# Chenxu1103/UNET-

Measured on AMD Instinct MI355X. Metric: frames/sec 512x512 3-class UNet++ inference; mask vs CPU reference, higher is better.
Workload: dtype f16 (MFMA operands split hi+lo, 3 MFMAs per product, f32 accumulate); 1 GPU; UNet++ 3-class 512x512 batch=16/GPU fp16-MFMA on 1 MI355X, synthetic frames, f32 NCHW in HBM -> uint8 mask in HBM; arch=nested, precision=exact, frames_per_gpu=16, global_batch=16, micro_batch=16, parallelism=frame-sharded x1, weights replicated (RCCL bcast)

## Files before the change

__graft_entry__.py:

```python
import os
import sys

ROOT = os.path.dirname(os.path.abspath(__file__))
if ROOT not in sys.path:
    sys.path.insert(0, ROOT)


def build() -> None:
    import unet_amd.nested_unet
    from unet_amd import _lib
    path = _lib.build(force=bool(os.environ.get("UNETPP_FORCE_BUILD")), verbose=True)
    import ctypes
    _lib.share_torch_hip_runtime()
    lib = ctypes.CDLL(path)
    for sym in _lib.ABI_SYMBOLS:
        getattr(lib, sym)
    print("built", path, "-", lib.unetpp_version.__name__, "ok")


def smoke() -> None:
    import numpy as np
    import torch
    from unet_amd import synthetic
    from unet_amd.nested_unet import NestedUNet
    sys.path.insert(0, os.path.join(ROOT, "oracle"))
    import unetpp_oracle as oracle

    assert torch.cuda.is_available(), "smoke() needs a HIP device"
    sd = synthetic.make_state_dict(3, 3, True, 2)
    frames = synthetic.make_frames_u8(2, 64, 96, "smooth", 7)
    x = synthetic.frames_to_chw_f32(frames)
    ref = oracle.torch_forward(sd, x)
    ref_mask, _, _ = oracle.masks_from_logits(ref)
    model = NestedUNet(3, deep_supervision=True, pretrained_encoder=False, max_batch=2, max_hw=(64, 96)).to("cuda:0")
    model.load_state_dict(sd, strict=True)
    model.eval()
    xt = torch.from_numpy(x).to("cuda:0")
    mask, logits = model.segment(xt, return_logits=True)
    torch.cuda.synchronize()
    err = float(np.abs(logits.cpu().numpy() - ref).max())
    margin = oracle.top2_margin(ref)
    bad = (mask.cpu().numpy() != ref_mask) & (margin > 1e-4)
    print(f"smoke: max|dlogit|={err:.3e} mask mismatches outside near-ties={int(bad.sum())}")
    assert err < 1e-3 and not bad.any()
    m8 = NestedUNet(3, deep_supervision=True, precision="exact8", max_batch=2, max_hw=(64, 96)).to("cuda:0")
    m8.load_state_dict(sd, strict=True)
    mask8, logits8 = m8.eval().segment(xt, return_logits=True)
    torch.cuda.synchronize()
    err8 = float(np.abs(logits8.cpu().numpy() - ref).max())
    bad8 = (mask8.cpu().numpy() != ref_mask) & (margin > 2 * err8 + 1e-7)
    print(f"smoke exact8: max|dlogit|={err8:.3e} mask mismatches outside near-ties={int(bad8.sum())}")
    assert err8 < 1e-3 and not bad8.any()


if __name__ == "__main__":
    build()
    if len(sys.argv) > 1 and sys.argv[1] == "smoke":
        smoke()
```

unet-_amd/_lib.py:

```python
from __future__ import annotations

import ctypes
import hashlib
import os
import shutil
import subprocess

_HERE = os.path.dirname(os.path.abspath(__file__))
LIB_PATH = os.path.join(_HERE, "libunetpp_hip.so")
CSRC = os.path.join(_HERE, "csrc")
SOURCES = ["unetpp_abi.hip"]
HEADERS = ["conv3x3_mfma.h", "conv3x3_ws.h", "tapmm_ws.h", "convt2x2_mfma.h", "aux_kernels.h", "components.h", "morphology.h", os.path.join("..", "..", "include", "unetpp.h")]

ABI_SYMBOLS = [
    "unetpp_create", "unetpp_destroy", "unetpp_last_error", "unetpp_version", "unetpp_weights_blob_bytes",
    "unetpp_weights_blob_bytes_arch",
    "unetpp_load_weights", "unetpp_load_weights_device", "unetpp_forward", "unetpp_forward_ex", "unetpp_mask_stats", "unetpp_workspace_bytes",
    "unetpp_resize_linear_u8", "unetpp_resize_nearest_roi_u8", "unetpp_status",
    "unetpp_profile_enable", "unetpp_profile_count", "unetpp_profile_read", "unetpp_profile_name",
    "unetpp_profile_work", "unetpp_debug_read", "unetpp_debug_keep_intermediates",
    "unetpp_ds_blob_bytes", "unetpp_load_ds_heads", "unetpp_forward_ds",
    "unetpp_components_workspace_bytes", "unetpp_components", "unetpp_components_filter",
    "unetpp_morphology", "unetpp_morphology_layout",
]

STATUS_OVERFLOW, STATUS_NAN = 1, 2
PREC_EXACT, PREC_FAST, PREC_EXACT8 = 0, 1, 2
PRECISIONS = {"exact": PREC_EXACT, "fast": PREC_FAST, "exact8": PREC_EXACT8}
ARCH_NESTED, ARCH_SIMPLE = 0, 1
IN_F32_NCHW, IN_U8_NHWC_BGR = 0, 1


class Config(ctypes.Structure):
    _fields_ = [("num_classes", ctypes.c_int), ("in_channels", ctypes.c_int), ("max_batch", ctypes.c_int),
                ("max_h", ctypes.c_int), ("max_w", ctypes.c_int), ("precision", ctypes.c_int),
                ("device", ctypes.c_int), ("micro_batch", ctypes.c_int), ("streams", ctypes.c_int), ("arch", ctypes.c_int)]


class CcRule(ctypes.Structure):
    _fields_ = [(n, ctypes.c_double) for n in ("min_area", "min_width", "max_width", "min_height_ratio", "min_aspect",
                                               "max_center_offset", "roi_width")]


CC_RULES = {"largest": 0, "spatial": 1, "cable_shape": 2}


class MorphElement(ctypes.Structure):
    _fields_ = [("kw", ctypes.c_int), ("kh", ctypes.c_int), ("ax", ctypes.c_int), ("ay", ctypes.c_int),
                ("host_data", ctypes.c_void_p)]


class MorphStep(ctypes.Structure):
    _fields_ = [(n, ctypes.c_int) for n in ("op", "dst", "a", "b", "element", "iterations")]


MORPH_OPS = {"dilate": 0, "erode": 1, "and": 2, "andnot": 3, "or": 4, "copy": 5}
RULES = {"argmax": 0, "thresholded_argmax": 1, "strict_bg_check": 2, "exclusive": 3}


class Outputs(ctypes.Structure):
    _fields_ = [("dev_logits", ctypes.c_void_p), ("dev_probs", ctypes.c_void_p), ("dev_mask", ctypes.c_void_p),
                ("dev_cable", ctypes.c_void_p), ("dev_tape", ctypes.c_void_p), ("rule", ctypes.c_int),
                ("t_cable", ctypes.c_float), ("t_tape", ctypes.c_float), ("bg_margin", ctypes.c_float),
                ("ct_margin", ctypes.c_float)]


CXXFLAGS = ["--offload-arch=gfx950", "-O3", "-std=c++17", "-fno-slp-vectorize"]


def source_hash() -> str:
    h = hashlib.sha256()
    h.update(" ".join(CXXFLAGS).encode() + b"\0")
    for rel in sorted(SOURCES + HEADERS):
        with open(os.path.join(CSRC, rel), "rb") as f:
            h.update(rel.encode() + b"\0" + f.read() + b"\0")
    return h.hexdigest()[:16]


def built_hash(path: str = LIB_PATH):
    try:
        with open(path, "rb") as f:
            blob = f.read()
    except OSError:
        return None
    i = blob.find(b"(gfx950) src:")
    if i < 0:
        return None
    tag = blob[i + 13:i + 13 + 16]
    if blob[i + 29:i + 36] == b" +wsdbg" and not os.environ.get("UNETPP_ALLOW_DBG_LIB"):
        return "wsdbg-build"
    return tag.decode("ascii", "replace")


def _stale() -> bool:
    return built_hash() != source_hash()


def _hipcc():
    cand = os.environ.get("HIPCC", "/opt/rocm/bin/hipcc")
    return cand if os.path.exists(cand) else shutil.which("hipcc")


def build(force: bool = False, verbose: bool = False) -> str:
    if not force and not _stale():
        return LIB_PATH
    hipcc = _hipcc()
    if not hipcc:
        raise RuntimeError("hipcc not found: cannot build libunetpp_hip.so")
    tmp = f"{LIB_PATH}.{os.getpid()}.tmp"
    cmd = [hipcc] + CXXFLAGS + ["-shared", "-fPIC", f'-DUNETPP_SRC_HASH="{source_hash()}"',
           "-o", tmp] + [os.path.join(CSRC, s) for s in SOURCES]
    if verbose:
        print(" ".join(cmd).replace(tmp, LIB_PATH), flush=True)
    try:
        subprocess.run(cmd, check=True, cwd=CSRC)
        os.replace(tmp, LIB_PATH)
    finally:
        if os.path.exists(tmp):
            os.remove(tmp)
    return LIB_PATH


_lib = None


def share_torch_hip_runtime() -> None:
    try:
        import torch
    except ImportError:
        pass


def load(build_if_missing: bool = True) -> ctypes.CDLL:
    global _lib
    if _lib is not None:
        return _lib
    share_torch_hip_runtime()
    if _stale():
        what = "is missing" if not os.path.exists(LIB_PATH) else f"was built from other sources (src:{built_hash()}, tree {source_hash()})"
        if not build_if_missing or not _hipcc():
            raise RuntimeError(f"{LIB_PATH} {what}: build it with __graft_entry__.build(); there is no CPU fallback")
        build()
    lib = ctypes.CDLL(LIB_PATH)
    vp, ci, cs = ctypes.c_void_p, ctypes.c_int, ctypes.c_size_t
    lib.unetpp_create.argtypes = [ctypes.POINTER(Config), ctypes.POINTER(vp)]; lib.unetpp_create.restype = ci
    lib.unetpp_destroy.argtypes = [vp]; lib.unetpp_destroy.restype = None
    lib.unetpp_last_error.argtypes = [vp]; lib.unetpp_last_error.restype = ctypes.c_char_p
    lib.unetpp_version.argtypes = []; lib.unetpp_version.restype = ctypes.c_char_p
    lib.unetpp_weights_blob_bytes.argtypes = [ci, ci]; lib.unetpp_weights_blob_bytes.restype = cs
    lib.unetpp_weights_blob_bytes_arch.argtypes = [ci, ci, ci]; lib.unetpp_weights_blob_bytes_arch.restype = cs
    lib.unetpp_load_weights.argtypes = [vp, vp, cs]; lib.unetpp_load_weights.restype = ci
    lib.unetpp_load_weights_device.argtypes = [vp, vp, cs, vp]; lib.unetpp_load_weights_device.restype = ci
    lib.unetpp_forward.argtypes = [vp, vp, ci, ci, ci, ci, vp, vp, vp, vp, vp]; lib.unetpp_forward.restype = ci
    lib.unetpp_forward_ex.argtypes = [vp, vp, ci, ci, ci, ci, ctypes.POINTER(Outputs), vp]; lib.unetpp_forward_ex.restype = ci
    lib.unetpp_mask_stats.argtypes = [vp, vp, ci, ci, ci, vp, vp, vp, vp]; lib.unetpp_mask_stats.restype = ci
    lib.unetpp_resize_linear_u8.argtypes = [vp, vp, ci, ci, ci, ci, vp, ci, ci, vp]; lib.unetpp_resize_linear_u8.restype = ci
    lib.unetpp_resize_nearest_roi_u8.argtypes = [vp, vp, ci, ci, ci, ci, vp, ci, ci, ci, ci, ci, ci, vp]
    lib.unetpp_resize_nearest_roi_u8.restype = ci
    lib.unetpp_workspace_bytes.argtypes = [vp]; lib.unetpp_workspace_bytes.restype = cs
    lib.unetpp_status.argtypes = [vp, ctypes.POINTER(ctypes.c_uint32), ci]; lib.unetpp_status.restype = ci
    lib.unetpp_profile_enable.argtypes = [vp, ci]; lib.unetpp_profile_enable.restype = ci
    lib.unetpp_profile_count.argtypes = [vp]; lib.unetpp_profile_count.restype = ci
    lib.unetpp_profile_read.argtypes = [vp, ctypes.POINTER(ctypes.c_float), ci]; lib.unetpp_profile_read.restype = ci
    lib.unetpp_profile_name.argtypes = [vp, ci]; lib.unetpp_profile_name.restype = ctypes.c_char_p
    lib.unetpp_profile_work.argtypes = [vp, ci, ctypes.POINTER(ctypes.c_double), ctypes.POINTER(ctypes.c_double)]
    lib.unetpp_profile_work.restype = ci
    lib.unetpp_debug_read.argtypes = [vp, ctypes.c_char_p, ctypes.POINTER(ctypes.c_float), cs]
    lib.unetpp_debug_read.restype = ctypes.c_longlong
    lib.unetpp_debug_keep_intermediates.argtypes = [vp, ci]; lib.unetpp_debug_keep_intermediates.restype = ci
    lib.unetpp_ds_blob_bytes.argtypes = [ci]; lib.unetpp_ds_blob_bytes.restype = cs
    lib.unetpp_load_ds_heads.argtypes = [vp, vp, cs]; lib.unetpp_load_ds_heads.restype = ci
    lib.unetpp_forward_ds.argtypes = [vp, vp, ci, ci, ci, ci, ctypes.POINTER(ctypes.POINTER(Outputs)), vp]
    lib.unetpp_forward_ds.restype = ci
# ... 18 lines not shown
```

unet-_amd/csrc/tapmm_ws.h:

```cpp
#pragma once
#include "conv3x3_ws.h"

namespace unetpp {

struct TapmmArgs {
  const half_t* low;
  const half_t* wpk;
  float* y;
  int N, hw, K, Nv;
#ifdef UNETPP_WS_DBG
  int dbg;
#endif
};

struct TapmmCfg {
  static constexpr int NT = 512, NCONS = 4, NPROD = 4;
  static constexpr int TM = 256, TN = 128, MT = 4, NTL = 2;
  static constexpr int A_BYTES = TM * 64, B_BYTES = TN * 64, STAGE_BYTES = A_BYTES + B_BYTES;
  static constexpr int SLOTS = 6, LDS_BYTES = SLOTS * STAGE_BYTES;
  static constexpr int A_PIECES = A_BYTES / 1024, B_PIECES = B_BYTES / 1024;
  static constexpr int A_IT = A_PIECES / NPROD, B_IT = B_PIECES / NPROD, DMA_PER_STAGE = A_IT + B_IT;
  static constexpr int AHEAD = 4;
  static_assert(LDS_BYTES <= 160 * 1024 && AHEAD + 2 <= SLOTS, "ring");
};

template <bool X8>
__global__ __launch_bounds__(512, 2) void tapmm_ws_kernel(TapmmArgs a) {
  using C = TapmmCfg;
  extern __shared__ __attribute__((aligned(16))) char smem[];
  touch_kernarg_lines<TapmmArgs>();
  const int tid = threadIdx.x, lane = tid & 63;
  const int wave = __builtin_amdgcn_readfirstlane(tid >> 6);
  const unsigned lds_base = (unsigned)(unsigned long)(lds_char_t*)smem;
  const int mtiles_img = (a.hw + C::TM - 1) / C::TM;
  const int ntiles = a.Nv / C::TN;
  const int total_tiles = a.N * mtiles_img * ntiles;
  const int nst = a.K / 16;
  const int G = (int)gridDim.x;
  const int slot = (G % 8 == 0) ? ((int)blockIdx.x % 8) * (G / 8) + (int)blockIdx.x / 8 : (int)blockIdx.x;
  auto decode = [&](int t, int& n, int& q0, int& vt) {
    vt = t % ntiles; t /= ntiles;
    const int mt = t % mtiles_img;
    n = t / mtiles_img;
    q0 = mt * C::TM;
  };
  if (slot >= total_tiles) return;
  if (wave >= C::NCONS) {
    const int pw = wave - C::NCONS;
    constexpr unsigned OOB = 0x80000000u;
    const unsigned blk_bytes = (unsigned)a.hw * 64u;
    int it_tile = slot, it_s = 0;
    int in_, iq0, ivt;
    decode(it_tile, in_, iq0, ivt);
    auto issue = [&](int ring) {
#ifdef UNETPP_WS_DBG
      if (a.dbg & 1) { if (++it_s == nst) { it_s = 0; it_tile += G; if (it_tile < total_tiles) decode(it_tile, in_, iq0, ivt); } return; }
#endif
      const __amdgpu_buffer_rsrc_t rs = __builtin_amdgcn_make_buffer_rsrc(
          (void*)(a.low + (size_t)in_ * (a.K / 16) * a.hw * 32), 0, (int)((a.K / 16) * blk_bytes), 0x00020000);
      const unsigned dstA = lds_base + ring * C::STAGE_BYTES;
#pragma unroll
      for (int it = 0; it < C::A_IT; ++it) {
        const int piece = pw + it * C::NPROD;
        const int q = iq0 + piece * 16 + (lane & 15);
        const unsigned voff = q < a.hw ? (unsigned)q * 64u + (unsigned)(lane >> 4) * 16u : OOB;
        blds16(rs, voff, it_s * (int)blk_bytes, dstA + piece * 1024);
      }
      const char* wsrc = (const char*)a.wpk + ((size_t)ivt * nst + it_s) * C::B_BYTES;
#pragma unroll
      for (int it = 0; it < C::B_IT; ++it) {
        const int piece = pw + it * C::NPROD;
        glds16(wsrc + piece * 1024, lane * 16, dstA + C::A_BYTES + piece * 1024);
      }
      if (++it_s == nst) {
        it_s = 0; it_tile += G;
        if (it_tile < total_tiles) decode(it_tile, in_, iq0, ivt);
      }
    };
    int issued = 0, g = 0;
    for (int k = 0; k <= C::AHEAD && it_tile < total_tiles; ++k, ++issued) issue(issued % C::SLOTS);
    for (int tile = slot; tile < total_tiles; tile += G)
      for (int s = 0; s < nst; ++s, ++g) {
        const int later = issued - (g + 2);
        if (later >= 3) asm volatile("s_waitcnt vmcnt(18)" ::: "memory");
        else if (later == 2) asm volatile("s_waitcnt vmcnt(12)" ::: "memory");
        else if (later == 1) asm volatile("s_waitcnt vmcnt(6)" ::: "memory");
        else asm volatile("s_waitcnt vmcnt(0)" ::: "memory");
        lds_barrier();
        if (it_tile < total_tiles) { issue(issued % C::SLOTS); ++issued; }
      }
    return;
  }

  const int cw = wave, pxh = cw & 1, vh = cw >> 1;
  static_assert(C::DMA_PER_STAGE == 6, "vmcnt ladder above");
  int a_off[C::MT];
#pragma unroll
  for (int mt = 0; mt < C::MT; ++mt) {
    const int px = pxh * 128 + mt * 32 + (lane & 31);
    a_off[mt] = (px >> 4) * 1024 + ((lane >> 5) * 16 + (px & 15)) * 16;
  }
  const int b_off = C::A_BYTES + (vh * 2) * 2048 + (lane >> 5) * 512 + (lane & 31) * 16;
  struct Frag { half8 ah[C::MT], al[C::MT], bh[C::NTL], bl[C::NTL]; };
  auto load_frags = [&](Frag& f, int ring) {
    const char* st = smem + ring * C::STAGE_BYTES;
#pragma unroll
    for (int mt = 0; mt < C::MT; ++mt) { f.ah[mt] = *(const half8*)(st + a_off[mt]); f.al[mt] = *(const half8*)(st + a_off[mt] + 512); }
#pragma unroll
    for (int nt = 0; nt < C::NTL; ++nt) { f.bh[nt] = *(const half8*)(st + b_off + nt * 2048); f.bl[nt] = *(const half8*)(st + b_off + nt * 2048 + 1024); }
  };
  float16v acc[C::MT][C::NTL];
  auto run_mfma = [&](const Frag& f) {
#ifdef UNETPP_WS_DBG
    if (a.dbg & 2) return;
#endif
#pragma unroll
    for (int mt = 0; mt < C::MT; ++mt)
#pragma unroll
      for (int nt = 0; nt < C::NTL; ++nt) {
        acc[mt][nt] = __builtin_amdgcn_mfma_f32_32x32x16_f16(f.bh[nt], f.al[mt], acc[mt][nt], 0, 0, 0);
        acc[mt][nt] = __builtin_amdgcn_mfma_f32_32x32x16_f16(f.bl[nt], f.ah[mt], acc[mt][nt], 0, 0, 0);
        acc[mt][nt] = __builtin_amdgcn_mfma_f32_32x32x16_f16(f.bh[nt], f.ah[mt], acc[mt][nt], 0, 0, 0);
      }
  };

  int g = 0;
  Frag f0, f1;
  bool have_f0 = false;
  struct HFrag { half8 a[C::MT], b[C::NTL]; };
  HFrag h0, h1;
  int8v xa[C::MT], xb[C::NTL];
  auto load_h = [&](HFrag& f, int ring) {
    const char* st = smem + ring * C::STAGE_BYTES;
#pragma unroll
    for (int mt = 0; mt < C::MT; ++mt) f.a[mt] = *(const half8*)(st + a_off[mt]);
#pragma unroll
    for (int nt = 0; nt < C::NTL; ++nt) f.b[nt] = *(const half8*)(st + b_off + nt * 2048);
  };
  auto load_x = [&](int ring0, int ring1) {
    const char* s0 = smem + ring0 * C::STAGE_BYTES;
    const char* s1 = smem + ring1 * C::STAGE_BYTES;
#pragma unroll
    for (int mt = 0; mt < C::MT; ++mt) {
      const int4v lo = *(const int4v*)(s0 + a_off[mt] + 512), hi = *(const int4v*)(s1 + a_off[mt] + 512);
      xa[mt] = __builtin_shufflevector(lo, hi, 0, 1, 2, 3, 4, 5, 6, 7);
    }
#pragma unroll
    for (int nt = 0; nt < C::NTL; ++nt) {
      const int4v lo = *(const int4v*)(s0 + b_off + nt * 2048 + 1024), hi = *(const int4v*)(s1 + b_off + nt * 2048 + 1024);
      xb[nt] = __builtin_shufflevector(lo, hi, 0, 1, 2, 3, 4, 5, 6, 7);
    }
  };
  auto main_mfma = [&](const HFrag& f) {
#pragma unroll
    for (int mt = 0; mt < C::MT; ++mt)
#pragma unroll
      for (int nt = 0; nt < C::NTL; ++nt) acc[mt][nt] = __builtin_amdgcn_mfma_f32_32x32x16_f16(f.b[nt], f.a[mt], acc[mt][nt], 0, 0, 0);
  };
  auto cross_mfma = [&]() {
#pragma unroll
    for (int mt = 0; mt < C::MT; ++mt)
#pragma unroll
      for (int nt = 0; nt < C::NTL; ++nt) {
        acc[mt][nt] = __builtin_amdgcn_mfma_scale_f32_32x32x64_f8f6f4(xb[nt], xa[mt], acc[mt][nt], 0 , 1 , 0, X8_SCALE_W, 0, X8_SCALE_A);
      }
  };
  for (int tile = slot; tile < total_tiles; tile += G) {
    int n, q0, vt;
    decode(tile, n, q0, vt);
#pragma unroll
    for (int mt = 0; mt < C::MT; ++mt)
#pragma unroll
      for (int nt = 0; nt < C::NTL; ++nt)
#pragma unroll
        for (int r = 0; r < 16; ++r) acc[mt][nt][r] = 0.f;
    const bool last_tile = tile + G >= total_tiles;
    if constexpr (X8) {
      for (int s = 0; s < nst; s += 2) {
        lds_barrier();
        if (!have_f0) { load_h(h0, g % C::SLOTS); have_f0 = true; }
        load_x(g % C::SLOTS, (g + 1) % C::SLOTS);
        load_h(h1, (g + 1) % C::SLOTS);
        __builtin_amdgcn_sched_barrier(0);
        main_mfma(h0);
        __builtin_amdgcn_sched_barrier(0);
        ++g;
        lds_barrier();
        const bool more = !(last_tile && s + 2 >= nst);
        if (more) load_h(h0, (g + 1) % C::SLOTS);
        have_f0 = more;
        __builtin_amdgcn_sched_barrier(0);
        cross_mfma();
        main_mfma(h1);
        __builtin_amdgcn_sched_barrier(0);
        ++g;
      }
    } else
    for (int s = 0; s < nst; s += 2) {
      lds_barrier();
      if (!have_f0) { load_frags(f0, g % C::SLOTS); have_f0 = true; }
      load_frags(f1, (g + 1) % C::SLOTS);
      __builtin_amdgcn_sched_barrier(0);
      run_mfma(f0);
      __builtin_amdgcn_sched_barrier(0);
      ++g;
      lds_barrier();
      const bool more = !(last_tile && s + 2 >= nst);
      if (more) load_frags(f0, (g + 1) % C::SLOTS);
      have_f0 = more;
      __builtin_amdgcn_sched_barrier(0);
      run_mfma(f1);
      __builtin_amdgcn_sched_barrier(0);
      ++g;
    }
#ifdef UNETPP_WS_DBG
    if (a.dbg & 4) { if (acc[0][0][0] == 12345.f) a.y[0] = 1.f; continue; }
#endif
    const int h = lane >> 5;
#pragma unroll
    for (int mt = 0; mt < C::MT; ++mt) {
      const int q = q0 + pxh * 128 + mt * 32 + (lane & 31);
#pragma unroll
      for (int nt = 0; nt < C::NTL; ++nt) {
        const int vb = vt * (C::TN / 32) + vh * 2 + nt;
        float* dst = a.y + (((size_t)n * (a.Nv / 32) + vb) * a.hw + q) * 32 + 4 * h;
        if (q < a.hw) {
#pragma unroll
          for (int qq = 0; qq < 4; ++qq) {
            typedef __attribute__((ext_vector_type(4))) float f32x4;
            *(f32x4*)(dst + 8 * qq) = (f32x4){acc[mt][nt][4 * qq], acc[mt][nt][4 * qq + 1], acc[mt][nt][4 * qq + 2], acc[mt][nt][4 * qq + 3]};
          }
        }
      }
    }
  }
}

__global__ void tapw_pack_kernel(const float* __restrict__ w, const float* __restrict__ mult, int Cout, int Cs, int Cup,
                                 half_t* __restrict__ out, long long units, int x8) {
  const long long u = (long long)blockIdx.x * blockDim.x + threadIdx.x;
  if (u >= units) return;
  long long t = u;
  const int vv = t % 32; t /= 32;
  const int kg = t % 2; t /= 2;
  const int pl = t % 2; t /= 2;
  const int vt = t % 4; t /= 4;
  const int nst = Cup / 16;
  const int ks = t % nst; t /= nst;
  const int v128 = (int)t;
  const int v = v128 * 128 + vt * 32 + vv;
  const int tap = v / Cout, co = v - tap * Cout;
  half8 r;
  float val[8];
#pragma unroll
  for (int e = 0; e < 8; ++e) {
    const int c = ks * 16 + kg * 8 + e;
    val[e] = w[((size_t)co * (Cs + Cup) + Cs + c) * 9 + tap] * mult[co];
    const half_t hi = (half_t)val[e];
    r[e] = pl == 0 ? hi : (half_t)(val[e] - (float)hi);
  }
  if (x8 && pl == 1) {
    unsigned wd[4];
#pragma unroll
    for (int q = 0; q < 2; ++q) {
      int a8 = 0, b8 = 0;
      float hi4[4], lo4[4];
#pragma unroll
      for (int i = 0; i < 4; ++i) { hi4[i] = val[4 * q + i] * 0.015625f; lo4[i] = (val[4 * q + i] - (float)(half_t)val[4 * q + i]) * 32.0f; }
      a8 = __builtin_amdgcn_cvt_pk_fp8_f32(hi4[0], hi4[1], a8, false); a8 = __builtin_amdgcn_cvt_pk_fp8_f32(hi4[2], hi4[3], a8, true);
      b8 = __builtin_amdgcn_cvt_pk_fp8_f32(lo4[0], lo4[1], b8, false); b8 = __builtin_amdgcn_cvt_pk_fp8_f32(lo4[2], lo4[3], b8, true);
      wd[2 * q] = (unsigned)a8; wd[2 * q + 1] = (unsigned)b8;
    }
    *(u32x4*)(out + u * 8) = (u32x4){wd[0], wd[1], wd[2], wd[3]};
    return;
  }
  *(half8*)(out + u * 8) = r;
}

struct UpsumArgs {
  const float* y;
  float* z;
  int N, H, W, Cout;
};

template <int TH_>
struct UpsumCfgT {
  static constexpr int TH = TH_, TW = 32, RH = TH / 2 + 3, RW = TW / 2 + 3, RECS = RH * RW;
  static constexpr int PIECES = (RECS * 128 + 1023) / 1024, BUF_BYTES = PIECES * 1024;
  static constexpr int YTAB_BYTES = (TH + 2) * 16, LDS_BYTES = BUF_BYTES + YTAB_BYTES;
  static constexpr int ITERS = (PIECES + 3) / 4;
};
typedef UpsumCfgT<16> UpsumCfg;

template <int TB, int TH_ = 16>
__global__ __launch_bounds__(256, TB == 1 ? 4 : 1) void upsum_kernel(UpsumArgs a) {
  using C = UpsumCfgT<TH_>;
  typedef __attribute__((ext_vector_type(4))) float f32x4;
  extern __shared__ __attribute__((aligned(16))) char smem[];
  const int H = a.H, W = a.W, h = H >> 1, w = W >> 1;
  const int tid = threadIdx.x, lane = tid & 63;
  const int wave = __builtin_amdgcn_readfirstlane(tid >> 6);
  const unsigned lds_base = (unsigned)(unsigned long)(lds_char_t*)smem;
  const int tiles_x = (W + C::TW - 1) / C::TW, tiles_y = (H + C::TH - 1) / C::TH;
  int t = blockIdx.x;
  const int tx = t % tiles_x; t /= tiles_x;
  const int ty = t % tiles_y; t /= tiles_y;
  const int cb = t % (a.Cout / 32);
  const int n = t / (a.Cout / 32);
  const int y0 = ty * C::TH, x0 = tx * C::TW;
  const float sh = h > 1 ? (float)(h - 1) / (float)(H - 1) : 0.f;
  const float sw = w > 1 ? (float)(w - 1) / (float)(W - 1) : 0.f;
  const int ybase = (int)(sh * (float)max(y0 - 1, 0)), xbase = (int)(sw * (float)max(x0 - 1, 0));
  const int vblocks = 9 * a.Cout / 32;
  const size_t plane = (size_t)h * w * 128;
  unsigned voff[C::ITERS];
#pragma unroll
  for (int it = 0; it < C::ITERS; ++it) {
    const int rec = (wave + it * 4) * 8 + (lane >> 3);
    const int ry = rec / C::RW, rx = rec - ry * C::RW;
    const int yy = min(ybase + ry, h - 1), xx = min(xbase + rx, w - 1);
    voff[it] = (wave + it * 4 < C::PIECES) ? (unsigned)((yy * w + xx) * 128 + (lane & 7) * 16) : 0x80000000u;
  }
  auto stage = [&](int tap, int buf) {
    const int vb = (tap * a.Cout) / 32 + cb;
    const __amdgpu_buffer_rsrc_t rs = __builtin_amdgcn_make_buffer_rsrc((void*)((const char*)a.y + ((size_t)n * vblocks + vb) * plane), 0,
                                                                       (int)plane, 0x00020000);
#pragma unroll
    for (int it = 0; it < C::ITERS; ++it) {
      const int piece = wave + it * 4;
      if (piece < C::PIECES) blds16(rs, voff[it], 0, lds_base + buf * C::BUF_BYTES + piece * 1024);
    }
  };
  const int cq = tid & 7, col = tid >> 3;
  int xo0[3], xo1[3]; float xl0[3], xl1[3];
#pragma unroll
  for (int dx = 0; dx < 3; ++dx) {
    const int xx = x0 + col + dx - 1;
    const bool in = xx >= 0 && xx < W && x0 + col < W;
    const float fx = sw * (float)max(xx, 0);
    const int c0 = min((int)fx, w - 1), c1 = c0 + (c0 < w - 1 ? 1 : 0);
    const float l1 = fminf(fmaxf(fx - (float)c0, 0.f), 1.f);
    xo0[dx] = min(max(c0 - xbase, 0), C::RW - 1) * 128 + cq * 16;
    xo1[dx] = min(max(c1 - xbase, 0), C::RW - 1) * 128 + cq * 16;
    xl0[dx] = in ? 1.f - l1 : 0.f; xl1[dx] = in ? l1 : 0.f;
  }
  struct YRow { int o0, o1; float l0, l1; };
  YRow* ytab = (YRow*)(smem + TB * C::BUF_BYTES);
  if (tid < C::TH + 2) {
    const int yy = y0 + tid - 1;
    const bool in = yy >= 0 && yy < H;
    const float fy = sh * (float)max(yy, 0);
    const int r0 = min((int)fy, h - 1), r1 = r0 + (r0 < h - 1 ? 1 : 0);
    const float l1 = fminf(fmaxf(fy - (float)r0, 0.f), 1.f);
    YRow e;
    e.o0 = min(max(r0 - ybase, 0), C::RH - 1) * (C::RW * 128);
    e.o1 = min(max(r1 - ybase, 0), C::RH - 1) * (C::RW * 128);
    e.l0 = in ? 1.f - l1 : 0.f; e.l1 = in ? l1 : 0.f;
// ... 41 lines not shown
```

unet-_amd/csrc/unetpp_abi.hip:

```cpp
#include <hip/hip_runtime.h>

#include <algorithm>
#include <cmath>
#include <cstdarg>
#include <cstdio>
#include <cstdlib>
#include <cstring>
#include <string>
#include <map>
#include <mutex>
#include <set>
#include <tuple>
#include <utility>
#include <vector>

#include "../../include/unetpp.h"
#include "aux_kernels.h"
#include "components.h"
#include "conv3x3_mfma.h"
#include "conv3x3_ws.h"
#include "convt2x2_mfma.h"
#include "morphology.h"
#include "tapmm_ws.h"

using namespace unetpp;

namespace {

thread_local std::string g_create_error;

constexpr uint32_t BLOB_MAGIC = 0x50504e55u;
constexpr uint32_t DS_BLOB_MAGIC = 0x53444e55u;
constexpr int BLOB_VERSION = 1;
const int NB[5] = {32, 64, 128, 256, 512};
const int SB[4] = {64, 128, 256, 512};

struct Tensor {
  std::string name;
  size_t off = 0;
  int C = 0;
  int lvl = 0;
  bool virt = false;
};

struct ConvLayer {
  std::string name;
  int cin_real = 0;
  int cout = 0;
  int lvl = 0;
  int in = -1, in2 = -1, out = -1, pool = -1;
  bool do_pool = false;
  int zt = -1;
  int y_t = -1, low_t = -1;
  half_t* tapw = nullptr;
  bool c0f = false;
  bool upf = false;
  bool ws = false;
  size_t w_off = 0, b_off = 0;
  int KC = 16, NW = 1, MW = 2, WAVES = 8;
  int nchunks = 1;
  half_t* wpk = nullptr;
  float* scale = nullptr;
  float* mult = nullptr;
};

struct ConvTLayer {
  std::string name;
  int cin = 0, cout = 0, lvl = 0;
  int in = -1, out = -1;
  size_t w_off = 0, b_off = 0;
  half_t* wpk = nullptr;
  float* scale = nullptr;
  float* mult = nullptr;
};

enum OpKind { OP_CONVERT, OP_CONV, OP_UP, OP_CONVT, OP_HEAD, OP_TAPMM, OP_UPSUM, OP_DS };
struct Op {
  OpKind kind;
  int idx = -1;
  int out = -1;
  bool fuse_head = false;
};

struct ProfRec {
  std::string name;
  double flops = 0, bytes = 0;
  int ev0 = -1, ev1 = -1;
};

}

struct unetpp_engine {
  unetpp_config cfg{};
  int P = 2;
  bool x8 = false;
  int mb = 1;
  int num_cus = 256;
  std::string err;
  char* arena = nullptr;
  size_t arena_bytes = 0;
  float* blob = nullptr;
  size_t blob_floats = 0;
  bool weights_loaded = false;
  std::vector<Tensor> tensors;
  std::vector<ConvLayer> convs;
  std::vector<ConvTLayer> convts;
  std::vector<Op> ops;
// ... 844 lines not shown
          return L.ws ? launch_ws(LaunchCtx{e->cfg.device, e->num_cus, e->ksplit_max, e->ksplit_min_chunks, e->ksplit_gate}, P, e->x8, a, L.do_pool, head, L.upf, L.c0f, s)
                    : launch_conv(LaunchCtx{e->cfg.device, e->num_cus}, P, L, mw, a, head, s);
        });
#ifdef UNETPP_WS_DBG
        if (stamp_this && L.ws) {
          static int printed = 0;
          std::vector<unsigned long long> hs(1024 * 32 * 5);
          (void)hipStreamSynchronize(s);
          (void)hipMemcpy(hs.data(), stamp_buf, hs.size() * 8, hipMemcpyDeviceToHost);
          if (printed++ == 3) {
            double sum[32] = {0};
            int nwg = 0;
            for (int b = 0; b < 1024; ++b) { if (!hs[b * 32 + 1] && !hs[b * 32 + 16]) continue; ++nwg; for (int i = 0; i < 32; ++i) sum[i] += (double)hs[b * 32 + i]; }
            fprintf(stderr, "[stamps %s] %d workgroups, mean cycles per workgroup:\n  consumer: barrier %.0f  chunks %.0f  epilogue %.0f  init %.0f\n"
                            "  producer: skip issue %.0f wait %.0f barrier %.0f | up issue %.0f interp %.0f (reads %.0f arithmetic %.0f split+stores %.0f) wait %.0f barrier %.0f | setup %.0f\n", L.name.c_str(), nwg,
                    sum[0] / nwg, sum[1] / nwg, sum[2] / nwg, sum[3] / nwg, sum[16] / nwg, sum[17] / nwg, sum[18] / nwg, sum[19] / nwg, sum[20] / nwg, sum[24] / nwg, sum[25] / nwg, sum[26] / nwg, sum[21] / nwg, sum[22] / nwg, sum[23] / nwg);
            std::vector<double> bg, en;
            unsigned long long t0 = ~0ull;
            std::vector<double> cb, pe;
            for (int b = 0; b < 1024; ++b) if (hs[b * 32 + 6]) t0 = std::min(t0, hs[b * 32 + 6]);
            for (int b = 0; b < 1024; ++b) if (hs[b * 32 + 6]) {
              bg.push_back((hs[b * 32 + 6] - t0) * 0.01); en.push_back((hs[b * 32 + 5] - t0) * 0.01);
              cb.push_back((hs[b * 32 + 4] - t0) * 0.01); pe.push_back((hs[b * 32 + 16 + 12] - t0) * 0.01);
            }
            std::sort(bg.begin(), bg.end()); std::sort(en.begin(), en.end()); std::sort(cb.begin(), cb.end()); std::sort(pe.begin(), pe.end());
            if (!bg.empty()) fprintf(stderr, "  consumer loop begins p50 %.2f max %.2f | producer wave 0 ends p50 %.2f max %.2f\n", cb[cb.size() / 2], cb.back(), pe[pe.size() / 2], pe.back());
            if (a.dbg & 131072)
              for (int b : {0, 1, 100, 200}) {
                for (int role = 0; role < 2; ++role) {
                  fprintf(stderr, "  wg %3d %s:", b, role ? "producer" : "consumer");
                  const unsigned long long* ev = hs.data() + 1024 * 32 + ((size_t)b * 2 + role) * 64;
                  for (int i = 0; i < 60 && ev[i]; ++i) fprintf(stderr, " %d:%.2f", (int)(ev[i] >> 56), (double)((ev[i] & 0xffffffffffffffull) - t0) * 0.01);
                  fprintf(stderr, "\n");
                }
              }
            if (!bg.empty())
              fprintf(stderr, "  wall clock (us after the first workgroup's kernel entry): entry p50 %.2f p90 %.2f max %.2f | end min %.2f p50 %.2f p90 %.2f max %.2f\n",
                      bg[bg.size() / 2], bg[bg.size() * 9 / 10], bg.back(), en.front(), en[en.size() / 2], en[en.size() * 9 / 10], en.back());
          }
        }
#endif
      } else if (op.kind == OP_TAPMM || op.kind == OP_UPSUM) {
        const ConvLayer& L = e->convs[op.idx];
        const int H = h >> L.lvl, W = w >> L.lvl;
        const int cs = e->tensors[L.in].C, cup = L.cin_real - cs;
        if (op.kind == OP_TAPMM) {
          TapmmArgs t{};
          t.low = tp(L.low_t); t.wpk = L.tapw; t.y = (float*)tp(L.y_t);
          t.N = nb; t.hw = (H >> 1) * (W >> 1); t.K = cup; t.Nv = 9 * L.cout;
#ifdef UNETPP_WS_DBG
          { const char* d = getenv("UNETPP_TAPMM_DBG"); t.dbg = d ? atoi(d) : 0; }
#endif
          const int tiles = nb * ((t.hw + TapmmCfg::TM - 1) / TapmmCfg::TM) * (t.Nv / TapmmCfg::TN);
          const double M = (double)nb * t.hw;
          char lbl[96];
          snprintf(lbl, sizeof lbl, "%s.up-gemm|tapmm_ws_kernel<%s>", L.name.c_str(), e->x8 ? "true" : "false");
          Lx.run(lbl, 2.0 * M * cup * t.Nv, M * cup * 2.0 * P + M * t.Nv * 4.0 + (double)t.Nv * cup * 2.0 * P, [&] {
            auto k = e->x8 ? tapmm_ws_kernel<true> : tapmm_ws_kernel<false>;
            hipError_t st = allow_full_lds((const void*)k, e->cfg.device);
            if (st != hipSuccess) return st;
            hipLaunchKernelGGL(k, dim3((unsigned)std::min(tiles, e->num_cus)), dim3(TapmmCfg::NT), TapmmCfg::LDS_BYTES, s, t);
            return hipSuccess;
          });
        } else {
          UpsumArgs u{};
          u.y = (const float*)tp(L.y_t); u.z = (float*)tp(L.zt); u.N = nb; u.H = H; u.W = W; u.Cout = L.cout;
          unsigned blocks = (unsigned)(((W + UpsumCfg::TW - 1) / UpsumCfg::TW) * ((H + UpsumCfg::TH - 1) / UpsumCfg::TH) * (L.cout / 32) * nb);
          const double px = (double)nb * H * W;
          char lbl[96];
          const bool small = blocks <= (unsigned)e->num_cus;
          if (small) blocks = (unsigned)(((W + 31) / 32) * ((H + 3) / 4) * (L.cout / 32) * nb);
          snprintf(lbl, sizeof lbl, "%s.up-sum|upsum_kernel<1, %d>", L.name.c_str(), small ? 4 : 16);
          Lx.run(lbl, px * L.cout * 9 * 8.0, px / 4 * 9 * L.cout * 4.0 + px * L.cout * 4.0, [&] {
            if (small) hipLaunchKernelGGL((upsum_kernel<1, 4>), dim3(blocks), dim3(256), UpsumCfgT<4>::LDS_BYTES, s, u);
            else hipLaunchKernelGGL((upsum_kernel<1, 16>), dim3(blocks), dim3(256), UpsumCfg::LDS_BYTES, s, u);
            return hipSuccess;
          });
        }
      } else if (op.kind == OP_UP) {
        const Tensor& low = e->tensors[op.idx];
        const Tensor& dst = e->tensors[op.out];
        const int H = h >> dst.lvl, W = w >> dst.lvl;
        double px = (double)nb * H * W;
        double bytes = px * P * 2.0 * low.C + px / 4 * P * 2.0 * low.C;
        const int nseg = (W + UP_SEG - 1) / UP_SEG;
        const int seg_w = std::min(W, UP_SEG);
        const size_t up_lds = (size_t)3 * (seg_w / 2 + 2) * P * 32;
        const int up_threads = seg_w * 2 * P >= 1024 ? 512 : (seg_w * 2 * P >= 256 ? 256 : 128);
        char nm[64];
        snprintf(nm, sizeof nm, "up%d|upsample2x_kernel<1>", dst.lvl);
        Lx.run(nm, px * low.C * 8, bytes, [&] {
          if (P != 1) return hipErrorInvalidValue;
          hipLaunchKernelGGL(upsample2x_kernel<1>, dim3((unsigned)((H / 2) * nseg), (unsigned)(nb * (low.C / 16))), dim3(up_threads), up_lds, s, tp(op.idx), H, W, tp(op.out));
          return hipSuccess;
        });
      } else if (op.kind == OP_CONVT) {
        ConvTLayer& T = e->convts[op.idx];
        ConvTArgs a{};
        const int H = h >> T.lvl, W = w >> T.lvl;
        a.in = tp(T.in); a.wpk = T.wpk; a.scale = T.scale; a.bias = e->blob + T.b_off; a.out = tp(T.out);
        a.N = nb; a.H = H; a.W = W; a.Cin = T.cin; a.Cout = T.cout;
        a.status = e->d_status;
        double px = (double)nb * H * W;
        double flops = 2.0 * px * T.cin * T.cout * 4;
        double bytes = px * P * 2.0 * (T.cin + 4.0 * T.cout) + 4.0 * T.cin * T.cout * 2.0 * P;
        dim3 grid((unsigned)(((H * W + 511) / 512) * (4 * T.cout / 64) * nb));
        char lbl[96];
        if (e->x8) snprintf(lbl, sizeof lbl, "%s|convt2x2_kernel<2, true>", T.name.c_str());
        else snprintf(lbl, sizeof lbl, "%s|convt2x2_kernel<%d>", T.name.c_str(), P);
        Lx.run(lbl, flops, bytes, [&] {
          if (e->x8) hipLaunchKernelGGL((convt2x2_kernel<2, true>), grid, dim3(256), 0, s, a);
          else if (P == 2) hipLaunchKernelGGL(convt2x2_kernel<2>, grid, dim3(256), 0, s, a);
          else hipLaunchKernelGGL(convt2x2_kernel<1>, grid, dim3(256), 0, s, a);
          return hipSuccess;
        });
      } else if (op.kind == OP_DS) {
        const int k = op.idx;
        const unetpp_outputs* dk = outs[k];
        if (!dk) continue;
// ... 559 lines not shown
```

Baseline: 3960 frames/s.

## Schedule tapmm tiles in XCD-aware panels and remap upsum blocks per XCD

Changes the persistent tapmm kernel's tile walk so that each XCD handles contiguous runs of tiles, grouped into column panels chosen on the host by a cost model of distinct A rows and B columns touched per XCD per round. The aim is better L2 reuse of activations and weights within each XCD's private cache. The upsum kernel also remaps blockIdx so that consecutive tiles land on the same XCD. It adds a debug-library build path and a Python model of the walks, and costs extra index arithmetic per tile plus a one-time host search.

```diff
diff --git a/__graft_entry__.py b/__graft_entry__.py
--- a/__graft_entry__.py
+++ b/__graft_entry__.py
@@ -10,6 +10,7 @@
     import unet_amd.nested_unet
     from unet_amd import _lib
     path = _lib.build(force=bool(os.environ.get("UNETPP_FORCE_BUILD")), verbose=True)
+    _lib.build_dbg(force=bool(os.environ.get("UNETPP_FORCE_BUILD")), verbose=True)
     import ctypes
     _lib.share_torch_hip_runtime()
     lib = ctypes.CDLL(path)
diff --git a/unet-_amd/_lib.py b/unet-_amd/_lib.py
--- a/unet-_amd/_lib.py
+++ b/unet-_amd/_lib.py
@@ -8,6 +8,7 @@
 
 _HERE = os.path.dirname(os.path.abspath(__file__))
 LIB_PATH = os.path.join(_HERE, "libunetpp_hip.so")
+DBG_LIB_PATH = os.path.join(_HERE, "libunetpp_hip_wsdbg.so")
 CSRC = os.path.join(_HERE, "csrc")
 SOURCES = ["unetpp_abi.hip"]
 HEADERS = ["conv3x3_mfma.h", "conv3x3_ws.h", "tapmm_ws.h", "convt2x2_mfma.h", "aux_kernels.h", "components.h", "morphology.h", os.path.join("..", "..", "include", "unetpp.h")]
@@ -77,7 +78,8 @@
     return h.hexdigest()[:16]
 
 
-def built_hash(path: str = LIB_PATH):
+def built_hash(path: str = None):
+    path = path or LIB_PATH
     try:
         with open(path, "rb") as f:
             blob = f.read()
@@ -101,24 +103,55 @@
     return cand if os.path.exists(cand) else shutil.which("hipcc")
 
 
+def _compile(out: str, defines, verbose: bool) -> str:
+    hipcc = _hipcc()
+    if not hipcc:
+        raise RuntimeError(f"hipcc not found: cannot build {os.path.basename(out)}")
+    tmp = f"{out}.{os.getpid()}.tmp"
+    cmd = [hipcc] + CXXFLAGS + ["-shared", "-fPIC"] + list(defines) + [f'-DUNETPP_SRC_HASH="{source_hash()}"',
+           "-o", tmp] + [os.path.join(CSRC, s) for s in SOURCES]
+    if verbose:
+        print(" ".join(cmd).replace(tmp, out), flush=True)
+    try:
+        subprocess.run(cmd, check=True, cwd=CSRC)
+        os.replace(tmp, out)
+    finally:
+        if os.path.exists(tmp):
+            os.remove(tmp)
+    return out
+
+
 def build(force: bool = False, verbose: bool = False) -> str:
     if not force and not _stale():
         return LIB_PATH
-    hipcc = _hipcc()
-    if not hipcc:
-        raise RuntimeError("hipcc not found: cannot build libunetpp_hip.so")
-    tmp = f"{LIB_PATH}.{os.getpid()}.tmp"
-    cmd = [hipcc] + CXXFLAGS + ["-shared", "-fPIC", f'-DUNETPP_SRC_HASH="{source_hash()}"',
-           "-o", tmp] + [os.path.join(CSRC, s) for s in SOURCES]
-    if verbose:
-        print(" ".join(cmd).replace(tmp, LIB_PATH), flush=True)
-    try:
-        subprocess.run(cmd, check=True, cwd=CSRC)
-        os.replace(tmp, LIB_PATH)
-    finally:
-        if os.path.exists(tmp):
-            os.remove(tmp)
-    return LIB_PATH
+    return _compile(LIB_PATH, [], verbose)
+
+
+def _dbg_built_hash():
+    try:
+        with open(DBG_LIB_PATH, "rb") as f:
+            blob = f.read()
+    except OSError:
+        return None
+    i = blob.find(b"(gfx950) src:")
+    if i < 0 or blob[i + 29:i + 36] != b" +wsdbg":
+        return None
+    return blob[i + 13:i + 13 + 16].decode("ascii", "replace")
+
+
+def build_dbg(force: bool = False, verbose: bool = False) -> str:
+    if not force and _dbg_built_hash() == source_hash():
+        return DBG_LIB_PATH
+    return _compile(DBG_LIB_PATH, ["-DUNETPP_WS_DBG=1"], verbose)
+
+
+def use_dbg_library() -> None:
+    global LIB_PATH
+    if _lib is not None:
+        raise RuntimeError("use_dbg_library() after the library was loaded")
+    build_dbg()
+    LIB_PATH = DBG_LIB_PATH
+    os.environ["UNETPP_ALLOW_DBG_LIB"] = "1"
 
 
 _lib = None
diff --git a/unet-_amd/csrc/tapmm_ws.h b/unet-_amd/csrc/tapmm_ws.h
--- a/unet-_amd/csrc/tapmm_ws.h
+++ b/unet-_amd/csrc/tapmm_ws.h
@@ -1,4 +1,5 @@
 #pragma once
+#include <vector>
 #include "conv3x3_ws.h"
 
 namespace unetpp {
@@ -8,10 +9,71 @@
   const half_t* wpk;
   float* y;
   int N, hw, K, Nv;
+  int pw, npan;
 #ifdef UNETPP_WS_DBG
   int dbg;
 #endif
 };
+
+__host__ __device__ inline int xcd_run_index(int b, int nblk) {
+  const int q = nblk / 8, r = nblk % 8, x = b % 8;
+  return (x < r ? x * (q + 1) : r * (q + 1) + (x - r) * q) + b / 8;
+}
+
+__host__ __device__ inline int tapmm_tile_of(int b, int G, int rnd, int total) {
+  const int full = total / G, rem = total - full * G;
+  if (rnd < full) return rnd * G + xcd_run_index(b, G);
+  if (rnd == full && b < rem) return full * G + xcd_run_index(b, rem);
+  return total;
+}
+
+__host__ __device__ inline void tapmm_decode(int t, int rows, int ntiles, int pw, int npan, int& row, int& vt) {
+  const int per_panel = rows * pw;
+  int p = t / per_panel;
+  if (p > npan - 1) p = npan - 1;
+  t -= p * per_panel;
+  const int c0 = p * pw, wd = p == npan - 1 ? ntiles - c0 : pw;
+  row = t / wd;
+  vt = c0 + (t - row * wd);
+}
+
+struct TapmmWalkCost { long worst, sum; };
+inline TapmmWalkCost tapmm_walk_cost(int rows, int ntiles, int pw, int npan, int G) {
+  const int total = rows * ntiles;
+  std::vector<int> seen_r((size_t)rows, -1), seen_c((size_t)ntiles, -1);
+  TapmmWalkCost c{0, 0};
+  for (int rnd = 0, stamp = 0; rnd * G < total; ++rnd)
+    for (int x = 0; x < 8; ++x, ++stamp) {
+      long here = 0;
+      for (int b = x; b < G; b += 8) {
+        const int t = tapmm_tile_of(b, G, rnd, total);
+        if (t >= total) continue;
+        int row, vt;
+        tapmm_decode(t, rows, ntiles, pw, npan, row, vt);
+        if (seen_r[row] != stamp) { seen_r[row] = stamp; here += 2; }
+        if (seen_c[vt] != stamp) { seen_c[vt] = stamp; here += 1; }
+      }
+      c.sum += here;
+      if (here > c.worst) c.worst = here;
+    }
+  return c;
+}
+
+inline void tapmm_choose_panels(int rows, int ntiles, int G, int& pw, int& npan) {
+  pw = ntiles; npan = 1;
+  if (G % 8 != 0) return;
+  const int W = G / 8;
+  const TapmmWalkCost base = tapmm_walk_cost(rows, ntiles, ntiles, 1, G);
+  TapmmWalkCost best = base;
+  for (int nb = 1; nb <= W && nb < ntiles; ++nb) {
+    if (W % nb != 0 || rows % (W / nb) != 0) continue;
+    for (int np = ntiles / nb; np <= (ntiles + nb - 1) / nb; ++np) {
+      const TapmmWalkCost c = tapmm_walk_cost(rows, ntiles, nb, np, G);
+      if (c.sum > base.sum) continue;
+      if (c.worst < best.worst || (c.worst == best.worst && c.sum < best.sum)) { best = c; pw = nb; npan = np; }
+    }
+  }
+}
 
 struct TapmmCfg {
   static constexpr int NT = 512, NCONS = 4, NPROD = 4;
@@ -37,24 +99,32 @@
   const int total_tiles = a.N * mtiles_img * ntiles;
   const int nst = a.K / 16;
   const int G = (int)gridDim.x;
-  const int slot = (G % 8 == 0) ? ((int)blockIdx.x % 8) * (G / 8) + (int)blockIdx.x / 8 : (int)blockIdx.x;
+  auto tile_of = [&](int rnd) {
+#ifdef UNETPP_WS_DBG
+    if (a.dbg & 8) {
+      const int slot = (G % 8 == 0) ? ((int)blockIdx.x % 8) * (G / 8) + (int)blockIdx.x / 8 : (int)blockIdx.x;
+      return min(slot + rnd * G, total_tiles);
+    }
+#endif
+    return tapmm_tile_of((int)blockIdx.x, G, rnd, total_tiles);
+  };
   auto decode = [&](int t, int& n, int& q0, int& vt) {
-    vt = t % ntiles; t /= ntiles;
-    const int mt = t % mtiles_img;
-    n = t / mtiles_img;
-    q0 = mt * C::TM;
-  };
-  if (slot >= total_tiles) return;
+    int row;
+    tapmm_decode(t, a.N * mtiles_img, ntiles, a.pw, a.npan, row, vt);
+    n = row / mtiles_img;
+    q0 = (row - n * mtiles_img) * C::TM;
+  };
+  if (tile_of(0) >= total_tiles) return;
   if (wave >= C::NCONS) {
     const int pw = wave - C::NCONS;
     constexpr unsigned OOB = 0x80000000u;
     const unsigned blk_bytes = (unsigned)a.hw * 64u;
-    int it_tile = slot, it_s = 0;
+    int it_rnd = 0, it_tile = tile_of(0), it_s = 0;
     int in_, iq0, ivt;
     decode(it_tile, in_, iq0, ivt);
     auto issue = [&](int ring) {
 #ifdef UNETPP_WS_DBG
-      if (a.dbg & 1) { if (++it_s == nst) { it_s = 0; it_tile += G; if (it_tile < total_tiles) decode(it_tile, in_, iq0, ivt); } return; }
+      if (a.dbg & 1) { if (++it_s == nst) { it_s = 0; it_tile = tile_of(++it_rnd); if (it_tile < total_tiles) decode(it_tile, in_, iq0, ivt); } return; }
 #endif
       const __amdgpu_buffer_rsrc_t rs = __builtin_amdgcn_make_buffer_rsrc(
           (void*)(a.low + (size_t)in_ * (a.K / 16) * a.hw * 32), 0, (int)((a.K / 16) * blk_bytes), 0x00020000);
@@ -73,13 +143,13 @@
         glds16(wsrc + piece * 1024, lane * 16, dstA + C::A_BYTES + piece * 1024);
       }
       if (++it_s == nst) {
-        it_s = 0; it_tile += G;
+        it_s = 0; it_tile = tile_of(++it_rnd);
         if (it_tile < total_tiles) decode(it_tile, in_, iq0, ivt);
       }
     };
     int issued = 0, g = 0;
     for (int k = 0; k <= C::AHEAD && it_tile < total_tiles; ++k, ++issued) issue(issued % C::SLOTS);
-    for (int tile = slot; tile < total_tiles; tile += G)
+    for (int rnd = 0; tile_of(rnd) < total_tiles; ++rnd)
       for (int s = 0; s < nst; ++s, ++g) {
         const int later = issued - (g + 2);
         if (later >= 3) asm volatile("s_waitcnt vmcnt(18)" ::: "memory");
@@ -165,7 +235,7 @@
         acc[mt][nt] = __builtin_amdgcn_mfma_scale_f32_32x32x64_f8f6f4(xb[nt], xa[mt], acc[mt][nt], 0 , 1 , 0, X8_SCALE_W, 0, X8_SCALE_A);
       }
   };
-  for (int tile = slot; tile < total_tiles; tile += G) {
+  for (int rnd = 0, tile; (tile = tile_of(rnd)) < total_tiles; ++rnd) {
     int n, q0, vt;
     decode(tile, n, q0, vt);
 #pragma unroll
@@ -174,7 +244,7 @@
       for (int nt = 0; nt < C::NTL; ++nt)
 #pragma unroll
         for (int r = 0; r < 16; ++r) acc[mt][nt][r] = 0.f;
-    const bool last_tile = tile + G >= total_tiles;
+    const bool last_tile = tile_of(rnd + 1) >= total_tiles;
     if constexpr (X8) {
       for (int s = 0; s < nst; s += 2) {
         lds_barrier();
@@ -281,6 +351,9 @@
   const float* y;
   float* z;
   int N, H, W, Cout;
+#ifdef UNETPP_WS_DBG
+  int dbg;
+#endif
 };
 
 template <int TH_>
@@ -302,7 +375,10 @@
   const int wave = __builtin_amdgcn_readfirstlane(tid >> 6);
   const unsigned lds_base = (unsigned)(unsigned long)(lds_char_t*)smem;
   const int tiles_x = (W + C::TW - 1) / C::TW, tiles_y = (H + C::TH - 1) / C::TH;
-  int t = blockIdx.x;
+  int t = xcd_run_index((int)blockIdx.x, (int)gridDim.x);
+#ifdef UNETPP_WS_DBG
+  if (a.dbg & 8) t = blockIdx.x;
+#endif
   const int tx = t % tiles_x; t /= tiles_x;
   const int ty = t % tiles_y; t /= tiles_y;
   const int cb = t % (a.Cout / 32);
diff --git a/unet-_amd/csrc/unetpp_abi.hip b/unet-_amd/csrc/unetpp_abi.hip
--- a/unet-_amd/csrc/unetpp_abi.hip
+++ b/unet-_amd/csrc/unetpp_abi.hip
@@ -53,6 +53,7 @@
   int zt = -1;
   int y_t = -1, low_t = -1;
   half_t* tapw = nullptr;
+  mutable int walk_tiles = -1, walk_grid = -1, walk_pw = 0, walk_npan = 1;
   bool c0f = false;
   bool upf = false;
   bool ws = false;
@@ -1003,6 +1004,15 @@
           { const char* d = getenv("UNETPP_TAPMM_DBG"); t.dbg = d ? atoi(d) : 0; }
 #endif
           const int tiles = nb * ((t.hw + TapmmCfg::TM - 1) / TapmmCfg::TM) * (t.Nv / TapmmCfg::TN);
+          const int grid = std::min(tiles, e->num_cus);
+          if (L.walk_tiles != tiles || L.walk_grid != grid) {
+            tapmm_choose_panels(tiles / (t.Nv / TapmmCfg::TN), t.Nv / TapmmCfg::TN, grid, L.walk_pw, L.walk_npan);
+            L.walk_tiles = tiles; L.walk_grid = grid;
+          }
+          t.pw = L.walk_pw; t.npan = L.walk_npan;
+#ifdef UNETPP_WS_DBG
+          if (t.dbg & 8) { t.pw = t.Nv / TapmmCfg::TN; t.npan = 1; }
+#endif
           const double M = (double)nb * t.hw;
           char lbl[96];
           snprintf(lbl, sizeof lbl, "%s.up-gemm|tapmm_ws_kernel<%s>", L.name.c_str(), e->x8 ? "true" : "false");
@@ -1010,12 +1020,15 @@
             auto k = e->x8 ? tapmm_ws_kernel<true> : tapmm_ws_kernel<false>;
             hipError_t st = allow_full_lds((const void*)k, e->cfg.device);
             if (st != hipSuccess) return st;
-            hipLaunchKernelGGL(k, dim3((unsigned)std::min(tiles, e->num_cus)), dim3(TapmmCfg::NT), TapmmCfg::LDS_BYTES, s, t);
+            hipLaunchKernelGGL(k, dim3((unsigned)grid), dim3(TapmmCfg::NT), TapmmCfg::LDS_BYTES, s, t);
             return hipSuccess;
           });
         } else {
           UpsumArgs u{};
           u.y = (const float*)tp(L.y_t); u.z = (float*)tp(L.zt); u.N = nb; u.H = H; u.W = W; u.Cout = L.cout;
+#ifdef UNETPP_WS_DBG
+          { const char* d = getenv("UNETPP_TAPMM_DBG"); u.dbg = d ? atoi(d) : 0; }
+#endif
           unsigned blocks = (unsigned)(((W + UpsumCfg::TW - 1) / UpsumCfg::TW) * ((H + UpsumCfg::TH - 1) / UpsumCfg::TH) * (L.cout / 32) * nb);
           const double px = (double)nb * H * W;
           char lbl[96];
diff --git a/unet-_amd/tile_walks.py b/unet-_amd/tile_walks.py
--- /dev/null
+++ b/unet-_amd/tile_walks.py
@@ -0,0 +1,96 @@
+from __future__ import annotations
+
+XCDS = 8
+TM, TN = 256, 128
+UPSUM_TW = 32
+
+
+def xcd_run_index(b: int, nblk: int) -> int:
+    q, r, x = nblk // XCDS, nblk % XCDS, b % XCDS
+    return (x * (q + 1) if x < r else r * (q + 1) + (x - r) * q) + b // XCDS
+
+
+def tapmm_tile_of(b: int, G: int, rnd: int, total: int) -> int:
+    full = total // G
+    rem = total - full * G
+    if rnd < full:
+        return rnd * G + xcd_run_index(b, G)
+    if rnd == full and b < rem:
+        return full * G + xcd_run_index(b, rem)
+    return total
+
+
+def tapmm_tile_of_before(b: int, G: int, rnd: int, total: int) -> int:
+    slot = (b % XCDS) * (G // XCDS) + b // XCDS if G % XCDS == 0 else b
+    return min(slot + rnd * G, total)
+
+
+def tapmm_decode(t: int, rows: int, ntiles: int, pw: int, npan: int):
+    per_panel = rows * pw
+    p = min(t // per_panel, npan - 1)
+    t -= p * per_panel
+    c0 = p * pw
+    wd = ntiles - c0 if p == npan - 1 else pw
+    row = t // wd
+    return row, c0 + (t - row * wd)
+
+
+def tapmm_xcd_rounds(rows: int, ntiles: int, pw: int, npan: int, G: int, tile_of=tapmm_tile_of):
+    total = rows * ntiles
+    out = []
+    rnd = 0
+    while rnd * G < total:
+        for x in range(XCDS):
+            tiles = [tile_of(b, G, rnd, total) for b in range(x, G, XCDS)]
+            cells = [tapmm_decode(t, rows, ntiles, pw, npan) for t in tiles if t < total]
+            if cells:
+                out.append((rnd, x, cells))
+        rnd += 1
+    return out
+
+
+def tapmm_walk_cost(rows: int, ntiles: int, pw: int, npan: int, G: int, tile_of=tapmm_tile_of):
+    per = [2 * len({r for r, _ in cells}) + len({c for _, c in cells})
+           for _, _, cells in tapmm_xcd_rounds(rows, ntiles, pw, npan, G, tile_of)]
+    return max(per), sum(per)
+
+
+def tapmm_choose_panels(rows: int, ntiles: int, G: int):
+    best = (ntiles, 1)
+    if G % XCDS:
+        return best
+    W = G // XCDS
+    base = best_cost = tapmm_walk_cost(rows, ntiles, ntiles, 1, G)
+    for nb in range(1, min(W, ntiles - 1) + 1):
+        if W % nb or rows % (W // nb):
+            continue
+        for np_ in range(ntiles // nb, -(-ntiles // nb) + 1):
+            c = tapmm_walk_cost(rows, ntiles, nb, np_, G)
+            if c[1] <= base[1] and c < best_cost:
+                best_cost, best = c, (nb, np_)
+    return best
+
+
+def upsum_tile(b: int, nblk: int, tiles_x: int, tiles_y: int, cblocks: int):
+    t = xcd_run_index(b, nblk)
+    tx, t = t % tiles_x, t // tiles_x
+    ty, t = t % tiles_y, t // tiles_y
+    return tx, ty, t % cblocks, t // cblocks
+
+
+def decoder_launches(batch: int, height: int, width: int, num_cus: int = 256):
+    nb_filter = (32, 64, 128, 256, 512)
+    out = []
+    for lvl in (2, 3):
+        H, W = height >> lvl, width >> lvl
+        cout, cup = nb_filter[lvl], nb_filter[lvl + 1]
+        hw = (H // 2) * (W // 2)
+        rows, ntiles = batch * ((hw + TM - 1) // TM), 9 * cout // TN
+        th = 16
+        blocks = ((W + UPSUM_TW - 1) // UPSUM_TW) * ((H + th - 1) // th) * (cout // 32) * batch
+        if blocks <= num_cus:
+            th = 4
+            blocks = ((W + UPSUM_TW - 1) // UPSUM_TW) * ((H + th - 1) // th) * (cout // 32) * batch
+        out.append({"level": lvl, "gemm": (rows, ntiles, cup, min(rows * ntiles, num_cus)),
+                    "upsum": ((W + UPSUM_TW - 1) // UPSUM_TW, (H + th - 1) // th, cout // 32, blocks), "th": th})
+    return out
```

After: 3982 frames/s (median of 6 runs). About the same (+0.5%).
